# bayespy/bayespy

Hardware: AMD Instinct MI355X
Metric: VB iterations/sec, PCA N=10000000 D=128 K=32 (higher is better)
Workload: dtype f64

## Files before the change

bayespy_amd/csrc/vmp_pca.hip:

```cpp
#include "vmp_common.h"
#include "vmp_stop_rule.h"

namespace {

constexpr int TN = 32;
constexpr int SZ = TN + 2;
constexpr int NT = 256;
constexpr int MAX_KP = 64;
constexpr int MAX_DP = 256;

inline int pow2_blocks(int x, int unit)
{
    int b = (x + unit - 1) / unit;
    int p = 1;
    while (p < b) p <<= 1;
    return p;
}

inline void fill_layout(int D, int K, vmp_pca_layout *L)
{
    const int64_t DP = 32 * pow2_blocks(D, 32);
    const int64_t KP = 16 * pow2_blocks(K, 16);
    int64_t o = 0;
    L->DP = DP;
// ... 1101 lines not shown
        return VMP_PCA_SWEEPS_NOT_BUILT;
    if (vmp_pca_sweep_covered(D, K) != VMP_OK) return VMP_PCA_SWEEPS_NOT_BUILT;
    VMP_REQUIRE(ctx, ring && order, VMP_ERR_INVALID, "null pointer argument");
    VMP_REQUIRE(ctx, n >= 1 && n <= VMP_PCA_MAX_SWEEPS, VMP_ERR_INVALID,
                "between 1 and %d sweeps per call", VMP_PCA_MAX_SWEEPS);
    VMP_REQUIRE(ctx, norder >= 1 && norder <= VMP_BOUND_MAX_ORDER, VMP_ERR_INVALID,
                "between 1 and %d bound terms", VMP_BOUND_MAX_ORDER);
    for (int i = 0; i < norder; ++i)
        VMP_REQUIRE(ctx, order[i] >= -1 && order[i] < VMP_BOUND_TERMS, VMP_ERR_INVALID,
                    "bound term %d out of range", order[i]);
    VMP_REQUIRE(ctx, lay == 0 || lay == 1 || lay == 3, VMP_ERR_INVALID, "unknown layout %d", lay);
    VMP_REQUIRE(ctx, x_prec > 0 && a0_tau > 0 && b0_tau > 0 && a0_alpha > 0 && b0_alpha > 0,
                VMP_ERR_INVALID, "x_prec and the Gamma prior parameters must be positive");
    int32_t rc;
    if (lay == 0) {
        rc = check_pass_args(ctx, Y, X, state, workspace, ldy, ldx, N, D, K);
        if (rc != VMP_OK) return rc;
    } else {
        VMP_REQUIRE(ctx, Y && X && state && workspace && N >= 0, VMP_ERR_INVALID,
                    "null pointer argument");
        VMP_REQUIRE(ctx, ((uintptr_t)Y % 16) == 0 && ((uintptr_t)X % 16) == 0, VMP_ERR_INVALID,
                    "tile-major arrays must be 16-byte aligned");
        if (lay == 1)
            VMP_REQUIRE(ctx, (ldx % 2) == 0 && ldx >= (N + TN - 1) / TN * TN && ldx < (int64_t)170000000,
                        VMP_ERR_INVALID, "row-major X beside a tile-major Y needs KP rows of an even "
                        "leading dimension >= 32 ceil(N/32) (ldx=%lld)", (long long)ldx);
    }
    rc = vmp_pca_ensure_gram(ctx);
    if (rc != VMP_OK) return rc;
    if (!ctx->sweep_ctl) {
        VMP_HIP_CHECK(ctx, hipMalloc(&ctx->sweep_ctl, VMP_SWEEP_CTL_LEN * sizeof(double)));
        VMP_HIP_CHECK(ctx, hipMemsetAsync(ctx->sweep_ctl, 0, VMP_SWEEP_CTL_LEN * sizeof(double),
                                          ctx->stream));
    }
    vmp_pca_layout L;
    fill_layout(D, K, &L);
    double *P = reinterpret_cast<double *>(workspace);
    vmp_sweep_tail t;
    t.P = P;
    t.nb = (int)(L.DP / GR);
    t.ctl = ctx->sweep_ctl;
    t.compare = compare ? 1 : 0;
    t.l0 = l0;
    t.tol = tol;
    t.norder = norder;
    for (int i = 0; i < 8; ++i) t.order[i] = i < norder ? order[i] : -1;
    const bool ticket = n > 1 && ((uintptr_t)state % 16) == 0 &&
                        vmp_tune_get("pca_sweep_ticket", env_int("VMP_PCA_SWEEP_TICKET", 1, 0, 1));
    int wide = vmp_tune_get("pca_sweep_wide", env_int("VMP_PCA_SWEEP_WIDE", 1, 0, 1)) ? 1 : 0;
    if (wide && vmp_tune_get("pca_sweep_local_pxx", env_int("VMP_PCA_SWEEP_LOCAL_PXX", 1, 0, 1)))
        wide = 2;
    if (wide == 2 && vmp_tune_get("pca_sweep_defer", env_int("VMP_PCA_SWEEP_DEFER", 1, 0, 1)))
        wide = 3;
    if (ticket && wide == 3) {
        rc = vmp_pca_sweep_constants(ctx, D, K, n_total, x_prec, a0_tau, b0_tau, a0_alpha, b0_alpha);
        if (rc != VMP_OK) return rc;
    }
    const int stamp_level = ticket ? vmp_tune_get("pca_sweep_stamps", 0) : 0;
    const bool stamps = stamp_level != 0;
    if (stamps) {
        const size_t bytes = (size_t)VMP_PCA_MAX_SWEEPS * VMP_SWEEP_NSTAMP * sizeof(unsigned long long);
        if (!ctx->sweep_stamps) VMP_HIP_CHECK(ctx, hipMalloc(&ctx->sweep_stamps, bytes));
        VMP_HIP_CHECK(ctx, hipMemsetAsync(ctx->sweep_stamps, 0,
                                          (size_t)(n - 1) * VMP_SWEEP_NSTAMP * sizeof(unsigned long long),
                                          ctx->stream));
        ctx->sweep_stamp_rows = n - 1;
    }
    if (ticket) {
        if (!ctx->sweep_tickets) {
            VMP_HIP_CHECK(ctx, hipMalloc(&ctx->sweep_tickets,
                                         VMP_PCA_MAX_SWEEPS * sizeof(unsigned int)));
            VMP_HIP_CHECK(ctx, hipMemsetAsync(ctx->sweep_tickets, 0,
                                              VMP_PCA_MAX_SWEEPS * sizeof(unsigned int), ctx->stream));
        }
    }
    bool head_wide = ticket && wide;
    if (head_wide && ctx->x_pending) {
        head_wide = hipEventQuery(ctx->ev_xdone) == hipSuccess;
        (void)hipGetLastError();
    }
    for (int i = 0; i < n; ++i) {
        const double *stop = i == 0 ? nullptr : ctx->sweep_ctl;
        const bool last = i + 1 == n;
        if (i == 0 && head_wide) {
            rc = vmp_pca_launch_sweep_head_wide(ctx, D, K, n_total, x_prec, a0_tau, b0_tau, a0_alpha,
                                                b0_alpha, state);
            if (rc != VMP_OK) return rc;
        } else if (!ticket || i == 0) {
            rc = vmp_pca_launch_sweep_head(ctx, D, K, n_total, x_prec, a0_tau, b0_tau, a0_alpha,
                                           b0_alpha, state, stop);
            if (rc != VMP_OK) return rc;
        }
        if (last) {
            rc = issue_xpass(ctx, Y, ldy, N, D, K, X, ldx, state, workspace, lay);
            if (rc != VMP_OK) return rc;
        } else {
            ctx->x_superseded += 1;
        }
        t.slot = ring + (int64_t)i * VMP_PCA_SWEEP_SLOT;
        t.first = i == 0;
        if (ticket && !last) {
            rc = vmp_pca_launch_sweep_mid(ctx, D, K, n_total, x_prec, a0_tau, b0_tau, a0_alpha,
                                          b0_alpha, state, P, t, ctx->sweep_tickets + i, wide,
                                          stamps ? ctx->sweep_stamps + (size_t)i * VMP_SWEEP_NSTAMP
                                                 : nullptr, stamp_level);
            if (rc != VMP_OK) return rc;
            ctx->sweep_mid_launches += 1;
        } else {
            rc = run_gram_stats(ctx, L, D, K, state, P, ctx->stream, stop, false);
            if (rc != VMP_OK) return rc;
            rc = vmp_pca_launch_sweep_tail(ctx, D, K, n_total, x_prec, a0_tau, b0_tau, a0_alpha,
                                           b0_alpha, state, t);
            if (rc != VMP_OK) return rc;
        }
        ctx->sweeps_enqueued += 1;
    }
    return VMP_OK;
}

int32_t vmp_pca_sweep_counts(vmp_ctx *ctx, int64_t *enqueued, int64_t *executed, int64_t *skipped)
{
    VMP_REQUIRE(ctx, ctx, VMP_ERR_INVALID, "null argument");
    double c[VMP_SWEEP_CTL_LEN] = {0.0};
    if (ctx->sweep_ctl) {
        VMP_HIP_CHECK(ctx, hipStreamSynchronize(ctx->stream));
        VMP_HIP_CHECK(ctx, hipMemcpy(c, ctx->sweep_ctl, sizeof(c), hipMemcpyDeviceToHost));
    }
    if (enqueued) *enqueued = ctx->sweeps_enqueued;
    if (executed) *executed = (int64_t)c[VMP_SWEEP_EXECUTED];
    if (skipped) *skipped = (int64_t)c[VMP_SWEEP_SKIPPED];
    return VMP_OK;
}

int32_t vmp_pca_sweep_mid_count(vmp_ctx *ctx, int64_t *launches)
{
    VMP_REQUIRE(ctx, ctx && launches, VMP_ERR_INVALID, "null argument");
    *launches = ctx->sweep_mid_launches;
    return VMP_OK;
}

int32_t vmp_pca_sweep_stamps(vmp_ctx *ctx, uint64_t *out, int32_t max_rows, int32_t *rows,
                             int32_t *allocated)
{
    VMP_REQUIRE(ctx, ctx && rows && max_rows >= 0 && (out || max_rows == 0), VMP_ERR_INVALID,
                "null argument");
    if (allocated) *allocated = ctx->sweep_stamps ? 1 : 0;
    *rows = 0;
    if (!ctx->sweep_stamps) return VMP_OK;
    const int n = ctx->sweep_stamp_rows < max_rows ? ctx->sweep_stamp_rows : max_rows;
    if (n > 0) {
        VMP_HIP_CHECK(ctx, hipStreamSynchronize(ctx->stream));
        VMP_HIP_CHECK(ctx, hipMemcpy(out, ctx->sweep_stamps,
                                     (size_t)n * VMP_SWEEP_NSTAMP * sizeof(unsigned long long),
                                     hipMemcpyDeviceToHost));
    }
    *rows = n;
    return VMP_OK;
}

int32_t vmp_pca_gram_stats_form(vmp_ctx *ctx, int32_t D, int32_t K, double *state, void *workspace,
                                int32_t form)
{
    VMP_REQUIRE(ctx, ctx && state && workspace, VMP_ERR_INVALID, "null argument");
    vmp_pca_layout L;
    const int32_t rc = vmp_pca_get_layout(D, K, &L);
    VMP_REQUIRE(ctx, rc == VMP_OK, rc, "unsupported dims D=%d K=%d", D, K);
    double *P = reinterpret_cast<double *>(workspace);
    if (form == 0) return run_gram_stats(ctx, L, D, K, state, P, ctx->stream, nullptr, false);
    VMP_REQUIRE(ctx, form == 1 || form == 2, VMP_ERR_INVALID, "form %d (0, 1 or 2)", form);
    return vmp_pca_launch_gram_fast(ctx, D, K, state, P, form == 2);
}

int32_t vmp_pca_last_pass_ms(vmp_ctx *ctx, double *ms_pass, double *ms_reduce)
{
    VMP_REQUIRE(ctx, ctx != nullptr, VMP_ERR_INVALID, "null argument");
    {
        const int32_t rch = vmp_pca_launch_held(ctx);
        if (rch != VMP_OK) return rch;
    }
    VMP_REQUIRE(ctx, ctx->timing && ctx->ev[0] && ctx->ev_n > 0, VMP_ERR_INVALID,
                "no timed pass (vmp_ctx_set_timing)");
    hipEvent_t *e = ctx->ev + 3 * ((ctx->ev_n - 1) % VMP_EV_RING);
    VMP_HIP_CHECK(ctx, hipEventSynchronize(e[2]));
    float a = 0.f, b = 0.f;
    VMP_HIP_CHECK(ctx, hipEventElapsedTime(&a, e[0], e[1]));
    VMP_HIP_CHECK(ctx, hipEventElapsedTime(&b, e[1], e[2]));
    if (ms_pass) *ms_pass = a;
    if (ms_reduce) *ms_reduce = b;
    return VMP_OK;
}

}
```

bayespy_amd/csrc/vmp_pca_small.hip:

```cpp
#include "vmp_common.h"
#include "vmp_sweep.h"
#include "vmp_stop_rule.h"

#include <stdlib.h>
#include <string.h>
#include <type_traits>

namespace {


struct small_args {
    vmp_pca_layout L;
    int D, K;
    double n_total, x_prec, a0t, b0t, a0a, b0a;
    int has_mean;
};

__device__ inline double ww_centred(const small_args &a, const double *st, int k)
{
    const vmp_pca_layout &L = a.L;
    double v = st[L.off_Sww + k * L.KP + k];
    if (a.has_mean) v += st[L.off_mstat + L.KP + k] - 2.0 * st[L.off_mstat + k];
    return v;
}
// ... 623 lines not shown
#pragma unroll
    for (int b = 0; b < NB; ++b)
#pragma unroll
        for (int m = 0; m < NLB; ++m) {
            const int e = tid + m * NTF;
            const int r = b * RB + e / KP, k = e % KP;
            wv[b][m] = (r < D && k < K) ? st[L.off_W + r * KP + k] : 0.0;
        }
#pragma unroll
    for (int b = 0; b < NB; ++b) {
        if (b < nb) {
#pragma unroll
            for (int m = 0; m < NLB; ++m) {
                const int e = tid + m * NTF;
                SWb[(e / KP) * LDM + (e % KP)] = wv[b][m];
            }
            __syncthreads();
#pragma unroll
            for (int t = 0; t < WT; ++t) {
                const int tile = w + 4 * t;
                if (tile < TPB) {
                    const int tk = tile % KT, td = tile / KT;
                    const v4f64 acc = wave_tile_mma(M + tk * 16 * LDM, LDM, 1, SWb + td * 16 * LDM, 1,
                                                    LDM, KP);
#pragma unroll
                    for (int r = 0; r < 4; ++r) {
                        const int k = tk * 16 + l4 + 4 * r, d = b * RB + td * 16 + l15;
                        if (k < K && d < D) st[L.off_A + k * DP + d] = tau * acc[r];
                    }
                }
            }
            __syncthreads();
        }
    }
    if (tid == 0) {
        st[L.off_scal + 1] = logdet;
        if (bad) st[L.off_scal + 3] = (double)VMP_ERR_NOT_POSDEF;
    }
    stamp.drain();
    stamp(SP_H_A);
}

template <int KP>
__global__ void __launch_bounds__(NTF, 5)
pca_head_fast_kernel(small_args a, double *st, const double *stop)
{
    if (stop && stop[VMP_SWEEP_STOP] != 0.0) return;
    pca_head_body<KP, false>(a, st, nullptr, nullptr, nullptr, 0.0);
}

constexpr int GB = 32;
constexpr int GRA = 8;
constexpr int TAIL_PLAIN = 0, TAIL_GRAM = 1, TAIL_SWEEP = 2;
template <int KP>
struct alignas(16) tail_lds {
    double Sw[KP * (KP + 1)];
    double Cx[KP * (KP + 1)];
    double Sx[KP * (KP + 1)];
    double al[4 * KP];
    double sc[8];
    double red[NTF / 64 + 1];
    double stop;
};
static_assert(sizeof(tail_lds<16>) % 16 == 0 && sizeof(tail_lds<32>) % 16 == 0, "tail_lds size");
template <int KP, int MODE, bool WIDE = false, class STAMP = stamps_off, bool LOCAL = false,
          bool DEFER = false>
__device__ __forceinline__ void pca_tail_body(const small_args &a, double *st, const vmp_sweep_tail *sw,
                                              tail_lds<KP> &s, double *SW = nullptr,
                                              const STAMP &stamp = STAMP(), const double *AL = nullptr)
{
    static_assert(!WIDE || MODE == TAIL_SWEEP, "the wide tail is a sweep tail");
    static_assert(!LOCAL || WIDE, "sum <x><x>^T is formed locally by the wide tail only");
    static_assert(!DEFER || LOCAL, "the bound is deferred behind the local wide tail only");
    constexpr bool GRAM = (MODE == TAIL_GRAM);
    constexpr int LDM = KP + 1, E = KP * KP / NTF;
    extern __shared__ __align__(16) double gl[];
    double *Sw = s.Sw, *Cx = s.Cx, *Sx = s.Sx, *al = s.al, *sc = s.sc, *red = s.red;
    const lay32 L(a.L);
    const int tid = threadIdx.x, D = a.D, K = a.K;
    if constexpr (MODE == TAIL_SWEEP && !LOCAL) {
        if (!sw->first && sw->ctl[VMP_SWEEP_STOP] != 0.0) {
            if (tid == 0) {
                sw->slot[7] = 0.0;
                sw->ctl[VMP_SWEEP_SKIPPED] += 1.0;
            }
            return;
        }
    }
    __builtin_amdgcn_s_setprio(3);
    double t1 = 0.0;
    double sxx[E];
#pragma unroll
    for (int m = 0; m < E; ++m) sxx[m] = 0.0;
    constexpr int NW = WIDE ? FAST_D * KP / NTF : 1;
    double ww[NW], wy[NW], es0[WIDE ? E : 1], es1[WIDE ? E : 1];
    if constexpr (WIDE) {
        const int n = D * KP;
#pragma unroll
        for (int j = 0; j < NW; ++j) {
            const int e = tid + j * NTF;
            ww[j] = e < n ? st[L.off_W + e] : 0.0;
            wy[j] = e < n ? st[L.off_S + e] : 0.0;
        }
#pragma unroll
        for (int m = 0; m < E; ++m) {
            const int e = tid + m * NTF;
            const int i = e / KP, j = e % KP;
            const bool in = (i < K && j < K);
            es0[m] = in ? st[L.off_Sww + i * KP + j] : 0.0;
            es1[m] = in ? st[L.off_CX + i * KP + j] : 0.0;
        }
    }
    if constexpr (LOCAL) {
    } else if constexpr (WIDE) {
        constexpr int NBM = FAST_D / 8;
        const int nb = sw->nb, nb4 = nb & ~3;
        double pv[E][NBM];
#pragma unroll
        for (int m = 0; m < E; ++m)
#pragma unroll
            for (int b = 0; b < NBM; ++b)
                pv[m][b] = b < nb ? sw->P[tid + m * NTF + b * (KP * KP)] : 0.0;
#pragma unroll
        for (int m = 0; m < E; ++m) {
            double s0 = 0.0, s1 = 0.0, s2 = 0.0, s3 = 0.0;
#pragma unroll
// ... 87 lines not shown
            const int i = e / KP, j = e % KP;
            const bool in = (i < K && j < K);
            if constexpr (WIDE) {
                v0[m] = es0[m];
                v1[m] = es1[m];
            } else {
                v0[m] = in ? st[L.off_Sww + i * KP + j] : 0.0;
                v1[m] = in ? st[L.off_CX + i * KP + j] : 0.0;
            }
            if constexpr (MODE != TAIL_PLAIN) v2[m] = in ? sxx[m] : 0.0;
            else v2[m] = in ? st[L.off_S + (L.DP + i) * KP + j] : 0.0;
        }
        if (tid == 0) {
            sc[4] = st[L.off_Syy];
            sc[5] = st[L.off_scal + 0];
            sc[6] = st[L.off_scal + 1];
        }
#pragma unroll
        for (int m = 0; m < E; ++m) {
            const int e = tid + m * NTF;
            const int i = e / KP, j = e % KP;
            Sw[i * LDM + j] = v0[m];
            Cx[i * LDM + j] = v1[m];
            if constexpr (!LOCAL) Sx[i * LDM + j] = v2[m];
        }
    }
    if constexpr (WIDE) {
        const int n = D * KP, jn = (n + 8 * NTF - 1) / (8 * NTF) * 8;
        const int nsw = LOCAL ? L.DP * KP : (D + 31) / 32 * 32 * KP;
#pragma unroll
        for (int j = 0; j < NW; ++j) {
            const int e = tid + j * NTF;
            if (j < jn) t1 += ww[j] * wy[j];
            if (e < nsw) SW[(e / KP) * LDM + (e % KP)] = (e < n && e % KP < K) ? wy[j] : 0.0;
        }
    } else if constexpr (!GRAM) {
        const int n = D * KP;
#pragma unroll 1
        for (int e0 = 0; e0 < n; e0 += 8 * NTF) {
            double w[8], y[8];
#pragma unroll
            for (int m = 0; m < 8; ++m) {
                const int e = e0 + tid + m * NTF;
                w[m] = e < n ? st[L.off_W + e] : 0.0;
                y[m] = e < n ? st[L.off_S + e] : 0.0;
            }
#pragma unroll
            for (int m = 0; m < 8; ++m) t1 += w[m] * y[m];
        }
    }
    (void)ww; (void)wy; (void)es0; (void)es1;
    __syncthreads();
    stamp(SP_T_LOADS);
    if constexpr (LOCAL) {
        constexpr int B = KP / 16;
        const int LA = L.DP + 2;
        const int ki = tid >> 4, ji = tid & 15;
        const int nb = sw->nb, nb4 = nb & ~3;
        const double *ar = AL + ki * LA, *sr = SW + ji;
        double acc[4][B][B];
#pragma unroll
        for (int q = 0; q < 4; ++q)
#pragma unroll
            for (int i = 0; i < B; ++i)
#pragma unroll
                for (int j = 0; j < B; ++j) acc[q][i][j] = 0.0;
        const auto group = [&](int b, double (&p)[B][B]) {
#pragma unroll
            for (int i = 0; i < B; ++i)
#pragma unroll
                for (int j = 0; j < B; ++j) p[i][j] = 0.0;
#pragma unroll
            for (int r = 0; r < GRA; r += 2) {
                v2f64 x[B];
                double y0[B], y1[B];
#pragma unroll
                for (int i = 0; i < B; ++i)
                    x[i] = *reinterpret_cast<const v2f64 *>(ar + 16 * i * LA + b * GRA + r);
#pragma unroll
                for (int j = 0; j < B; ++j) {
                    y0[j] = sr[(b * GRA + r) * LDM + 16 * j];
                    y1[j] = sr[(b * GRA + r + 1) * LDM + 16 * j];
                }
#pragma unroll
                for (int i = 0; i < B; ++i)
#pragma unroll
                    for (int j = 0; j < B; ++j) {
                        p[i][j] = __builtin_fma(x[i][0], y0[j], p[i][j]);
                        p[i][j] = __builtin_fma(x[i][1], y1[j], p[i][j]);
                    }
            }
        };
        double p[B][B];
#pragma unroll 1
        for (int b = 0; b < nb4; b += 4) {
#pragma unroll
            for (int q = 0; q < 4; ++q) {
                group(b + q, p);
#pragma unroll
                for (int i = 0; i < B; ++i)
#pragma unroll
                    for (int j = 0; j < B; ++j) acc[q][i][j] += p[i][j];
            }
        }
#pragma unroll 1
        for (int b = nb4; b < nb; ++b) {
            group(b, p);
// ... 218 lines not shown
        const double *a0 = As + k0 * LA, *a1 = As + (k0 + H) * LA;
        double s00 = 0.0, s01 = 0.0, s10 = 0.0, s11 = 0.0;
#pragma unroll 4
        for (int d = 0; d < D; ++d) {
            const double x0 = g0[d], x1 = g1[d], y0 = a0[d], y1 = a1[d];
            s00 = __builtin_fma(x0, y0, s00);
            s01 = __builtin_fma(x0, y1, s01);
            s10 = __builtin_fma(x1, y0, s10);
            s11 = __builtin_fma(x1, y1, s11);
        }
        Ss[ra * LDS_S + k0] = s00;
        Ss[ra * LDS_S + k0 + H] = s01;
        Ss[(ra + 4) * LDS_S + k0] = s10;
        Ss[(ra + 4) * LDS_S + k0 + H] = s11;
        double *So = st + L.off_S;
        if (r0 + ra < D) {
            if (k0 < K) So[(r0 + ra) * KP + k0] = s00;
            if (k0 + H < K) So[(r0 + ra) * KP + k0 + H] = s01;
        }
        if (r0 + ra + 4 < D) {
            if (k0 < K) So[(r0 + ra + 4) * KP + k0] = s10;
            if (k0 + H < K) So[(r0 + ra + 4) * KP + k0 + H] = s11;
        }
    }
    __syncthreads();
    stamp(SP_SYX);
    double *Pb = P + (int64_t)blk * KP * KP;
#pragma unroll
    for (int m = 0; m < E; ++m) {
        const int e = tid + m * NTF;
        const int k = e / KP, k2 = e % KP;
        double s = 0.0;
        if (k < K && k2 < K) {
#pragma unroll
            for (int r = 0; r < GRA; ++r) s = __builtin_fma(As[k * LA + r0 + r], Ss[r * LDS_S + k2], s);
        }
        Pb[e] = s;
    }
}

template <int KP>
__global__ void __launch_bounds__(NTF)
pca_gram_fast_kernel(vmp_pca_layout L, int D, int K, double *st, double *P)
{
    extern __shared__ __align__(16) double gl[];
    gram_phase_a<KP>(L, D, K, st, P, gl, blockIdx.x);
}

__host__ __device__ inline size_t gram_phase_a_wide_lds(int KP, int DP)
{
    return ((size_t)KP * (DP + 2) + (size_t)GRA * DP + (size_t)GRA * (KP + 1)) * sizeof(double);
}

template <int KP, class STAMP = stamps_off, bool PXX = true>
__device__ __forceinline__ void gram_phase_a_wide(const vmp_pca_layout &L, int D, int K, double *st,
                                                  double *P, double *lds, int blk,
                                                  const STAMP &stamp = STAMP())
{
    constexpr int LDS_S = KP + 1, KT = KP / 16, E = KP * KP / NTF;
    constexpr int NA = KP * (FAST_D / 2) / NTF, NG = GRA * (FAST_D / 2) / NTF;
    const int DP = (int)L.DP, LA = DP + 2;
    const int DP2 = DP >> 1, sh = __builtin_ctz(DP2);
    double *As = lds;
    double *Gs = As + KP * LA;
    double *Ss = Gs + GRA * DP;
    const int tid = threadIdx.x;
    const int r0 = blk * GRA;
    const double *A = st + L.off_A;
    const double *G = st + L.off_G + (int64_t)r0 * DP;
    v2f64 av[NA], gv[NG];
#pragma unroll
    for (int m = 0; m < NA; ++m) {
        const int e = tid + m * NTF;
        const int k = e >> sh, c = (e & (DP2 - 1)) * 2;
        av[m] = *reinterpret_cast<const v2f64 *>(A + (k < K ? k : K - 1) * DP + c);
    }
#pragma unroll
    for (int m = 0; m < NG; ++m) {
        const int e = tid + m * NTF;
        gv[m] = *reinterpret_cast<const v2f64 *>(G + 2 * (e < GRA * DP2 ? e : GRA * DP2 - 1));
    }
#pragma unroll
    for (int m = 0; m < NA; ++m) {
        const int e = tid + m * NTF;
        const int k = e >> sh, c = (e & (DP2 - 1)) * 2;
        if (e < KP * DP2) *reinterpret_cast<v2f64 *>(As + k * LA + c) = k < K ? av[m] : v2f64{0.0, 0.0};
    }
#pragma unroll
    for (int m = 0; m < NG; ++m) {
        const int e = tid + m * NTF;
        if (e < GRA * DP2) *reinterpret_cast<v2f64 *>(Gs + 2 * e) = gv[m];
    }
    __syncthreads();
    stamp(SP_LDS_FILLED);
    {
        const int w = tid >> 6, l = tid & 63;
        if (w < 2 * KT) {
            const int k = (l & 15) + 16 * (w % KT), r = (l >> 4) + 4 * (w / KT);
            const double *g = Gs + r * DP, *ar = As + k * LA;
            double s = 0.0;
#pragma unroll 16
            for (int d = 0; d < D; ++d) s = __builtin_fma(g[d], ar[d], s);
            Ss[r * LDS_S + k] = s;
            if (r0 + r < D && k < K) st[L.off_S + (r0 + r) * KP + k] = s;
        }
    }
    __syncthreads();
    stamp(SP_SYX);
    if constexpr (PXX) {
        double *Pb = P + (int64_t)blk * KP * KP;
#pragma unroll
        for (int m = 0; m < E; ++m) {
            const int e = tid + m * NTF;
            const int k = e / KP, k2 = e % KP;
            double s = 0.0;
            if (k < K && k2 < K) {
#pragma unroll
                for (int r = 0; r < GRA; ++r)
                    s = __builtin_fma(As[k * LA + r0 + r], Ss[r * LDS_S + k2], s);
            }
            Pb[e] = s;
        }
    }
}

template <int KP>
__global__ void __launch_bounds__(NTF)
pca_gram_wide_kernel(vmp_pca_layout L, int D, int K, double *st, double *P)
{
    extern __shared__ __align__(16) double gl[];
    gram_phase_a_wide<KP>(L, D, K, st, P, gl, blockIdx.x);
}

template <int KP, class STAMP>
struct defer_side {
    const small_args &a;
    double *st;
    const vmp_sweep_tail &sw;
    tail_lds<KP> &s;
    const double *sf;
    const STAMP &stamp;
    __device__ __forceinline__ void operator()() const
    {
        constexpr int LDM = KP + 1;
        if (threadIdx.x >= 128) return;
        const lay32 L(a.L);
        const int l = threadIdx.x - 64, D = a.D, K = a.K;
        const bool isa = l < K;
        const int k = isa ? l : 0;
        const double a0 = isa ? a.a0a : a.a0t, b0 = isa ? a.b0a : a.b0t;
        const double av = isa ? s.al[0 * KP + k] : s.sc[0];
        const double bv = isa ? s.al[1 * KP + k] : s.sc[1];
        const double mean = isa ? s.al[2 * KP + k] : s.sc[2];
        const double *c = sf + (isa ? VMP_SWEEP_SF_ALPHA : VMP_SWEEP_SF_TAU);
        const double dg = c[0], lga = c[1], lga0 = c[2], logb0 = c[3];
        const double logb = sf_log(bv);
        const double logx = dg - logb;
        const double g_p = a0 * logb0 - lga0;
        const double g_q = av * logb - lga;
        const double g = g_p - g_q + (bv - b0) * mean + (a0 - av) * logx;
        if (isa) st[L.off_alpha + 3 * KP + k] = logx;
        if (l == 32) st[L.off_tau + 3] = logx;
        stamp.side(SP_S_STATE);
        const double sla = 0.0 + wave_sum(isa ? logx : 0.0);
        const double saw = 0.0 + wave_sum(isa ? mean * s.Sw[k * LDM + k] : 0.0);
        const double lal = 0.0 + wave_sum(isa ? g : 0.0);
        const double logtau = __shfl(logx, 32, 64), Lt = __shfl(g, 32, 64);
        if (l == 0) {
            const double tau = s.sc[2], resid = s.red[0], trx = s.red[1];
            const double Dd = (double)D, Kd = (double)K;
            const double LY = Dd * a.n_total * (-0.5 * sf[VMP_SWEEP_SF_LOG2PI] + 0.5 * logtau)
                              - 0.5 * tau * resid;
            const double LX = -0.5 * a.x_prec * trx
                              + a.n_total * (0.5 * Kd * sf[VMP_SWEEP_SF_LOGXPREC] - 0.5 * s.sc[6] + 0.5 * Kd);
            const double LW = 0.5 * Dd * sla - 0.5 * saw + Dd * (-0.5 * s.sc[5] + 0.5 * Kd);
            st[L.off_L + 0] = LY;
            st[L.off_L + 1] = LX;
            st[L.off_L + 2] = LW;
            st[L.off_L + 3] = Lt;
            st[L.off_L + 4] = lal;
            st[L.off_L + 5] = LY + LX + LW + Lt + lal;
            const double status = !(s.sc[1] > 0.0) ? (double)VMP_ERR_FLOATING : st[L.off_scal + 3];
            double *slot = sw.slot;
            slot[0] = LY;
// ... 116 lines not shown
    }
    __syncthreads();
    stamp(SP_H_SWW);
#pragma unroll
    for (int m = 0; m < E; ++m) {
        const int e = tid + m * NTF;
        const int i = e / KP, j = e % KP;
        double x = (i == j) ? 1.0 : 0.0;
        if (i < K && j < K) {
            x = tau * 0.5 * (T[i * LDM + j] + T[j * LDM + i]);
            if (i == j) x += a.x_prec;
        }
        M[i * LDM + j] = x;
    }
    const auto pad = [&]() {
        if (D == nr && K == KP) return;
        for (int e = tid - 64; e < nr * KP; e += NTF - 64)
            if (e / KP >= D || e % KP >= K) SW[(e / KP) * LDM + (e % KP)] = 0.0;
    };
    sweep_inverse<KP>(M, K, &logdet, &bad, pad);
    stamp(SP_H_INV2);
#pragma unroll
    for (int m = 0; m < E; ++m) {
        const int e = tid + m * NTF;
        const int i = e / KP, j = e % KP;
        if (i < K && j < K) st[L.off_CX + i * KP + j] = M[i * LDM + j];
    }
#pragma unroll
    for (int t = 0; t < WT; ++t) {
        const int tile = w + 4 * t;
        if (tile < nt) {
            const int tk = tile % KT, td = tile / KT;
            const v4f64 acc = wave_tile_mma(M + tk * 16 * LDM, LDM, 1, SW + td * 16 * LDM, 1, LDM, KP);
#pragma unroll
            for (int r = 0; r < 4; ++r) {
                const int k = tk * 16 + l4 + 4 * r, d = td * 16 + l15;
                if (k < K && d < D) st[L.off_A + k * DP + d] = tau * acc[r];
            }
        }
    }
    if (tid == 0) {
        st[L.off_scal + 1] = logdet;
        if (bad) st[L.off_scal + 3] = (double)VMP_ERR_NOT_POSDEF;
    }
    stamp.drain();
    stamp(SP_H_A);
}

__host__ __device__ inline size_t sweep_local_lds(int KP, int DP)
{
    return ((size_t)KP * (DP + 2) + (size_t)DP * (KP + 1) + 2) * sizeof(double);
}

template <int KP, bool WIDE, bool LOCAL, bool DEFER, class STAMP>
__device__ __forceinline__ void pca_sweep_mid_body(const small_args &a, double *st, double *P,
                                                   const vmp_sweep_tail &sw, unsigned int *ticket,
                                                   const double *sf, const STAMP &stamp)
{
    static_assert(!LOCAL || WIDE, "sum <x><x>^T is formed locally beside the wide bodies only");
    static_assert(!DEFER || LOCAL, "the bound is deferred behind the local wide tail only");
    extern __shared__ __align__(16) double gl[];
    __shared__ tail_lds<KP> ts;
    const int tid = threadIdx.x;
    if (!sw.first && sw.ctl[VMP_SWEEP_STOP] != 0.0) {
        if (blockIdx.x == 0 && tid == 0) {
            sw.slot[7] = 0.0;
            sw.ctl[VMP_SWEEP_SKIPPED] += 1.0;
        }
        return;
    }
    stamp(SP_ENTRY);
    if constexpr (WIDE)
        gram_phase_a_wide<KP, STAMP, !LOCAL>(a.L, a.D, a.K, st, P, gl, blockIdx.x, stamp);
    else
        gram_phase_a<KP>(a.L, a.D, a.K, st, P, gl, blockIdx.x, stamp);
    asm volatile("s_waitcnt vmcnt(0)" ::: "memory");
    __syncthreads();
    stamp(SP_PXX);
    const int na = LOCAL ? KP * ((int)a.L.DP + 2) : 0;
    double *SW = gl + na;
    unsigned int *word = reinterpret_cast<unsigned int *>(LOCAL ? SW + (int)a.L.DP * (KP + 1) : gl);
    if (tid == 0) {
        __builtin_amdgcn_fence(__ATOMIC_RELEASE, "agent");
        asm volatile("s_waitcnt vmcnt(0)" ::: "memory");
        *word = __hip_atomic_fetch_add(ticket, 1u, __ATOMIC_RELAXED, __HIP_MEMORY_SCOPE_AGENT);
    }
    __syncthreads();
    if (*word != gridDim.x - 1) return;
    stamp(SP_TICKET);
    if (tid == 0) {
        __builtin_amdgcn_fence(__ATOMIC_ACQUIRE, "agent");
        asm volatile("s_waitcnt vmcnt(0)" ::: "memory");
        *ticket = 0u;
    }
    __syncthreads();
    stamp(SP_ACQUIRE);
    pca_tail_body<KP, TAIL_SWEEP, WIDE, STAMP, LOCAL, DEFER>(a, st, &sw, ts, SW, stamp, gl);
    __syncthreads();
    if constexpr (DEFER) {
        const defer_side<KP, STAMP> side{a, st, sw, ts, sf, stamp};
        pca_head_wide<KP>(a, st, ts.Cx, ts.Sx, ts.al + 2 * KP, ts.sc[2], SW, stamp, side, &ts.stop);
        return;
    }
    if (ts.stop != 0.0) return;
    if constexpr (WIDE)
        pca_head_wide<KP>(a, st, ts.Cx, ts.Sx, ts.al + 2 * KP, ts.sc[2], SW, stamp);
    else
        pca_head_body<KP, true>(a, st, ts.Cx, ts.Sx, ts.al + 2 * KP, ts.sc[2], stamp);
}

template <int KP, bool WIDE, bool LOCAL, bool DEFER = false>
__global__ void __launch_bounds__(NTF)
pca_sweep_mid_kernel(small_args a, double *st, double *P, vmp_sweep_tail sw, unsigned int *ticket,
                     const double *sf)
{
    pca_sweep_mid_body<KP, WIDE, LOCAL, DEFER>(a, st, P, sw, ticket, sf, stamps_off());
}

template <int KP, bool WIDE, bool LOCAL, bool DEFER = false>
__global__ void __launch_bounds__(NTF)
pca_sweep_mid_stamped_kernel(small_args a, double *st, double *P, vmp_sweep_tail sw,
                             unsigned int *ticket, const double *sf, unsigned long long *out, int level)
{
    __shared__ unsigned long long stl[VMP_SWEEP_NSTAMP];
    if (threadIdx.x < VMP_SWEEP_NSTAMP) stl[threadIdx.x] = 0;
    __syncthreads();
    const stamps_on stamp{stl, level};
    pca_sweep_mid_body<KP, WIDE, LOCAL, DEFER>(a, st, P, sw, ticket, sf, stamp);
    if (threadIdx.x == 0 && stl[SP_T_LOADS] != 0)
        for (int i = 0; i < VMP_SWEEP_NSTAMP; ++i) out[i] = stl[i];
}

template <int KP>
__global__ void __launch_bounds__(NTF)
pca_head_wide_kernel(small_args a, double *st)
{
    constexpr int LDM = KP + 1, E = KP * KP / NTF, NW = FAST_D * KP / NTF;
    __shared__ __align__(16) double M[KP * LDM], T[KP * LDM], SW[FAST_D * LDM], alm[KP];
    const lay32 L(a.L);
    const int tid = threadIdx.x, D = a.D, K = a.K;
    const int n = D * KP, nsw = (D + 31) / 32 * 32 * KP;
    double cx[E], sx[E], wy[NW];
#pragma unroll
    for (int m = 0; m < E; ++m) {
        const int e = tid + m * NTF;
        const int i = e / KP, j = e % KP;
        const bool in = (i < K && j < K);
        cx[m] = in ? st[L.off_CX + i * KP + j] : 0.0;
        sx[m] = in ? st[L.off_S + (L.DP + i) * KP + j] : 0.0;
    }
#pragma unroll
    for (int j = 0; j < NW; ++j) {
        const int e = tid + j * NTF;
        wy[j] = (e < n && e % KP < K) ? st[L.off_S + e] : 0.0;
    }
    const double tau = st[L.off_tau + 2];
    if (tid < KP) alm[tid] = tid < K ? st[L.off_alpha + 2 * KP + tid] : 0.0;
#pragma unroll
    for (int m = 0; m < E; ++m) {
        const int e = tid + m * NTF;
        M[(e / KP) * LDM + (e % KP)] = cx[m];
        T[(e / KP) * LDM + (e % KP)] = sx[m];
    }
#pragma unroll
    for (int j = 0; j < NW; ++j) {
        const int e = tid + j * NTF;
        if (e < nsw) SW[(e / KP) * LDM + (e % KP)] = wy[j];
    }
    __syncthreads();
    pca_head_wide<KP>(a, st, M, T, alm, tau, SW, stamps_off());
}

__global__ void __launch_bounds__(64)
pca_sweep_sf_kernel(small_args a, double *sf)
{
    const int l = threadIdx.x;
    if (l >= VMP_SWEEP_SF_LEN) return;
    const double ta = a.a0t + 0.5 * (double)a.D * a.n_total;
    const double aa = a.a0a + 0.5 * (double)a.D;
    double v;
    switch (l) {
// ... 161 lines not shown

int32_t vmp_pca_launch_sweep_head(vmp_ctx *ctx, int32_t D, int32_t K, int64_t n_total, double x_prec,
                                  double a0t, double b0t, double a0a, double b0a, double *state,
                                  const double *stop)
{
    small_args a;
    const int32_t rc = fill_small_args(ctx, a, D, K, n_total, x_prec, a0t, b0t, a0a, b0a);
    if (rc != VMP_OK) return rc;
    if (a.L.KP == 16)
        hipLaunchKernelGGL(pca_head_fast_kernel<16>, dim3(1), dim3(NTF), 0, ctx->stream, a, state, stop);
    else
        hipLaunchKernelGGL(pca_head_fast_kernel<32>, dim3(1), dim3(NTF), 0, ctx->stream, a, state, stop);
    VMP_HIP_CHECK(ctx, hipGetLastError());
    return VMP_OK;
}

int32_t vmp_pca_launch_sweep_tail(vmp_ctx *ctx, int32_t D, int32_t K, int64_t n_total, double x_prec,
                                  double a0t, double b0t, double a0a, double b0a, double *state,
                                  const vmp_sweep_tail &t)
{
    small_args a;
    const int32_t rc = fill_small_args(ctx, a, D, K, n_total, x_prec, a0t, b0t, a0a, b0a);
    if (rc != VMP_OK) return rc;
    if (a.L.KP == 16)
        hipLaunchKernelGGL(pca_tail_sweep_kernel<16>, dim3(1), dim3(NTF), 0, ctx->stream, a, state, t);
    else
        hipLaunchKernelGGL(pca_tail_sweep_kernel<32>, dim3(1), dim3(NTF), 0, ctx->stream, a, state, t);
    VMP_HIP_CHECK(ctx, hipGetLastError());
    return VMP_OK;
}

template <typename F>
static int32_t raise_lds_once(vmp_ctx *ctx, F *k16, F *k32, bool *raised)
{
    const int dev = ctx->device & 63;
    if (raised[dev]) return VMP_OK;
    VMP_HIP_CHECK(ctx, hipFuncSetAttribute((const void *)k16,
                                           hipFuncAttributeMaxDynamicSharedMemorySize, 96 * 1024));
    VMP_HIP_CHECK(ctx, hipFuncSetAttribute((const void *)k32,
                                           hipFuncAttributeMaxDynamicSharedMemorySize, 96 * 1024));
    raised[dev] = true;
    return VMP_OK;
}

int32_t vmp_pca_launch_gram_fast(vmp_ctx *ctx, int32_t D, int32_t K, double *state, double *P,
                                 int32_t wide)
{
    vmp_pca_layout L;
    const int32_t rc = vmp_pca_get_layout(D, K, &L);
    VMP_REQUIRE(ctx, rc == VMP_OK, rc, "unsupported dims D=%d K=%d", D, K);
    VMP_REQUIRE(ctx, L.KP <= 32 && D <= FAST_D, VMP_ERR_UNSUPPORTED,
                "the fast Gram statistics cover K <= 32, D <= %d", FAST_D);
    VMP_REQUIRE(ctx, ((uintptr_t)state % 16) == 0, VMP_ERR_INVALID, "state must be 16-byte aligned");
    static bool raised[2][64] = {{false}};
    const int32_t rr = wide ? raise_lds_once(ctx, pca_gram_wide_kernel<16>, pca_gram_wide_kernel<32>,
                                             raised[1])
                            : raise_lds_once(ctx, pca_gram_fast_kernel<16>, pca_gram_fast_kernel<32>,
                                             raised[0]);
    if (rr != VMP_OK) return rr;
    const int nb = (int)(L.DP / GRA);
    if (wide) {
        const size_t ldw = gram_phase_a_wide_lds((int)L.KP, (int)L.DP);
        if (L.KP == 16)
            hipLaunchKernelGGL(pca_gram_wide_kernel<16>, dim3(nb), dim3(NTF), ldw, ctx->stream, L, D, K,
                               state, P);
        else
            hipLaunchKernelGGL(pca_gram_wide_kernel<32>, dim3(nb), dim3(NTF), ldw, ctx->stream, L, D, K,
                               state, P);
        VMP_HIP_CHECK(ctx, hipGetLastError());
        return VMP_OK;
    }
    const size_t lds = gram_phase_a_lds((int)L.KP, (int)L.DP);
    if (L.KP == 16)
        hipLaunchKernelGGL(pca_gram_fast_kernel<16>, dim3(nb), dim3(NTF), lds, ctx->stream, L, D, K,
                           state, P);
    else
        hipLaunchKernelGGL(pca_gram_fast_kernel<32>, dim3(nb), dim3(NTF), lds, ctx->stream, L, D, K,
                           state, P);
    VMP_HIP_CHECK(ctx, hipGetLastError());
    return VMP_OK;
}

template <int KP, bool WIDE, bool LOCAL, bool DEFER = false>
static int32_t launch_mid(vmp_ctx *ctx, const small_args &a, double *state, double *P,
                          const vmp_sweep_tail &t, unsigned int *ticket, unsigned long long *stamps,
                          int stamp_level)
{
    VMP_REQUIRE(ctx, !DEFER || ctx->sweep_sf, VMP_ERR_INVALID,
                "the deferred sweep needs vmp_pca_sweep_constants first");
    static bool raised[2][64] = {{false}};
    const int dev = ctx->device & 63, s = stamps ? 1 : 0;
    if (!raised[s][dev]) {
        const void *f = stamps ? (const void *)pca_sweep_mid_stamped_kernel<KP, WIDE, LOCAL, DEFER>
                               : (const void *)pca_sweep_mid_kernel<KP, WIDE, LOCAL, DEFER>;
        VMP_HIP_CHECK(ctx, hipFuncSetAttribute(f, hipFuncAttributeMaxDynamicSharedMemorySize,
                                               96 * 1024));
        raised[s][dev] = true;
    }
    const size_t lds = LOCAL ? sweep_local_lds((int)a.L.KP, (int)a.L.DP)
                       : WIDE ? gram_phase_a_wide_lds((int)a.L.KP, (int)a.L.DP)
                              : gram_phase_a_lds((int)a.L.KP, (int)a.L.DP);
    const dim3 nb((unsigned)(a.L.DP / GRA));
    if (stamps)
        hipLaunchKernelGGL((pca_sweep_mid_stamped_kernel<KP, WIDE, LOCAL, DEFER>), nb, dim3(NTF), lds,
                           ctx->stream, a, state, P, t, ticket, (const double *)ctx->sweep_sf, stamps,
                           stamp_level);
    else
        hipLaunchKernelGGL((pca_sweep_mid_kernel<KP, WIDE, LOCAL, DEFER>), nb, dim3(NTF), lds, ctx->stream, a,
                           state, P, t, ticket, (const double *)ctx->sweep_sf);
    VMP_HIP_CHECK(ctx, hipGetLastError());
    return VMP_OK;
}

int32_t vmp_pca_launch_sweep_mid(vmp_ctx *ctx, int32_t D, int32_t K, int64_t n_total, double x_prec,
                                 double a0t, double b0t, double a0a, double b0a, double *state,
                                 double *P, const vmp_sweep_tail &t, unsigned int *ticket, int32_t wide,
                                 unsigned long long *stamps, int32_t stamp_level)
{
    small_args a;
    const int32_t rc = fill_small_args(ctx, a, D, K, n_total, x_prec, a0t, b0t, a0a, b0a);
    if (rc != VMP_OK) return rc;
    const int sl = stamp_level;
    if (a.L.KP == 16)
        return wide == 3 ? launch_mid<16, true, true, true>(ctx, a, state, P, t, ticket, stamps, sl)
               : wide == 2 ? launch_mid<16, true, true>(ctx, a, state, P, t, ticket, stamps, sl)
               : wide      ? launch_mid<16, true, false>(ctx, a, state, P, t, ticket, stamps, sl)
                           : launch_mid<16, false, false>(ctx, a, state, P, t, ticket, stamps, sl);
    return wide == 3 ? launch_mid<32, true, true, true>(ctx, a, state, P, t, ticket, stamps, sl)
           : wide == 2 ? launch_mid<32, true, true>(ctx, a, state, P, t, ticket, stamps, sl)
           : wide      ? launch_mid<32, true, false>(ctx, a, state, P, t, ticket, stamps, sl)
                       : launch_mid<32, false, false>(ctx, a, state, P, t, ticket, stamps, sl);
}

int32_t vmp_pca_sweep_constants(vmp_ctx *ctx, int32_t D, int32_t K, int64_t n_total, double x_prec,
                                double a0t, double b0t, double a0a, double b0a)
{
    small_args a;
    const int32_t rc = fill_small_args(ctx, a, D, K, n_total, x_prec, a0t, b0t, a0a, b0a);
    if (rc != VMP_OK) return rc;
    const double key[7] = {a0t, b0t, a0a, b0a, (double)D, (double)n_total, x_prec};
    if (ctx->sweep_sf && ctx->sweep_sf_valid && memcmp(key, ctx->sweep_sf_key, sizeof(key)) == 0)
        return VMP_OK;
    if (!ctx->sweep_sf) VMP_HIP_CHECK(ctx, hipMalloc(&ctx->sweep_sf, VMP_SWEEP_SF_LEN * sizeof(double)));
    ctx->sweep_sf_valid = 0;
    hipLaunchKernelGGL(pca_sweep_sf_kernel, dim3(1), dim3(64), 0, ctx->stream, a, ctx->sweep_sf);
    VMP_HIP_CHECK(ctx, hipGetLastError());
    memcpy(ctx->sweep_sf_key, key, sizeof(key));
    ctx->sweep_sf_valid = 1;
    return VMP_OK;
}

int32_t vmp_pca_launch_sweep_head_wide(vmp_ctx *ctx, int32_t D, int32_t K, int64_t n_total,
                                       double x_prec, double a0t, double b0t, double a0a, double b0a,
                                       double *state)
{
    small_args a;
    const int32_t rc = fill_small_args(ctx, a, D, K, n_total, x_prec, a0t, b0t, a0a, b0a);
    if (rc != VMP_OK) return rc;
    if (a.L.KP == 16)
        hipLaunchKernelGGL(pca_head_wide_kernel<16>, dim3(1), dim3(NTF), 0, ctx->stream, a, state);
    else
        hipLaunchKernelGGL(pca_head_wide_kernel<32>, dim3(1), dim3(NTF), 0, ctx->stream, a, state);
    VMP_HIP_CHECK(ctx, hipGetLastError());
    return VMP_OK;
}

extern "C" {

int32_t vmp_pca_small_ops(vmp_ctx *ctx, int32_t D, int32_t K, int64_t n_total, double x_prec,
                          double a0_tau, double b0_tau, double a0_alpha, double b0_alpha,
                          int32_t nops, const int32_t *ops, double *state)
{
    return launch_small(ctx, D, K, n_total, x_prec, a0_tau, b0_tau, a0_alpha, b0_alpha, nops, ops,
                        state);
}

int32_t vmp_pca_small_ops_mean(vmp_ctx *ctx, int32_t D, int32_t K, int64_t n_total, double x_prec,
                               double a0_tau, double b0_tau, double a0_alpha, double b0_alpha,
                               int32_t nops, const int32_t *ops, int32_t has_mean, double *state)
{
    return launch_small(ctx, D, K, n_total, x_prec, a0_tau, b0_tau, a0_alpha, b0_alpha, nops, ops,
// ... 40 lines not shown
```

Measured before the change: 26070.

## Add lean sweep path with padded Gram staging and register-tiled local Pxx

Adds a LEAN variant of the deferred wide sweep-mid kernel, on by default. It pads the staged Gram rows in LDS to stride DP+2 and reads them as v2f64 pairs in the A·G dot products, to cut LDS bank conflicts and load count. For KP=32 it also replaces the local sum <x><x>^T loop with a 4x4 register-tiled accumulation, reduced across lanes with DPP row swaps and shuffles. It exposes a standalone lean Gram kernel as form 3. The cost is a slightly larger LDS footprint, more register pressure and more template variants.

Result: no change. 26040 (median of 2 runs) (-0.1%).

```diff
diff --git a/bayespy_amd/csrc/vmp_pca.hip b/bayespy_amd/csrc/vmp_pca.hip
--- a/bayespy_amd/csrc/vmp_pca.hip
+++ b/bayespy_amd/csrc/vmp_pca.hip
@@ -1177,6 +1177,7 @@
         wide = 2;
     if (wide == 2 && vmp_tune_get("pca_sweep_defer", env_int("VMP_PCA_SWEEP_DEFER", 1, 0, 1)))
         wide = 3;
+    const bool lean = wide == 3 && vmp_tune_get("pca_sweep_lean", env_int("VMP_PCA_SWEEP_LEAN", 1, 0, 1));
     if (ticket && wide == 3) {
         rc = vmp_pca_sweep_constants(ctx, D, K, n_total, x_prec, a0_tau, b0_tau, a0_alpha, b0_alpha);
         if (rc != VMP_OK) return rc;
@@ -1226,7 +1227,8 @@
         t.first = i == 0;
         if (ticket && !last) {
             rc = vmp_pca_launch_sweep_mid(ctx, D, K, n_total, x_prec, a0_tau, b0_tau, a0_alpha,
-                                          b0_alpha, state, P, t, ctx->sweep_tickets + i, wide,
+                                          b0_alpha, state, P, t, ctx->sweep_tickets + i,
+                                          lean ? 4 : wide,
                                           stamps ? ctx->sweep_stamps + (size_t)i * VMP_SWEEP_NSTAMP
                                                  : nullptr, stamp_level);
             if (rc != VMP_OK) return rc;
@@ -1292,8 +1294,8 @@
     VMP_REQUIRE(ctx, rc == VMP_OK, rc, "unsupported dims D=%d K=%d", D, K);
     double *P = reinterpret_cast<double *>(workspace);
     if (form == 0) return run_gram_stats(ctx, L, D, K, state, P, ctx->stream, nullptr, false);
-    VMP_REQUIRE(ctx, form == 1 || form == 2, VMP_ERR_INVALID, "form %d (0, 1 or 2)", form);
-    return vmp_pca_launch_gram_fast(ctx, D, K, state, P, form == 2);
+    VMP_REQUIRE(ctx, form >= 1 && form <= 3, VMP_ERR_INVALID, "form %d (0, 1, 2 or 3)", form);
+    return vmp_pca_launch_gram_fast(ctx, D, K, state, P, form - 1);
 }
 
 int32_t vmp_pca_last_pass_ms(vmp_ctx *ctx, double *ms_pass, double *ms_reduce)
diff --git a/bayespy_amd/csrc/vmp_pca_small.hip b/bayespy_amd/csrc/vmp_pca_small.hip
--- a/bayespy_amd/csrc/vmp_pca_small.hip
+++ b/bayespy_amd/csrc/vmp_pca_small.hip
@@ -699,6 +699,13 @@
 constexpr int GB = 32;
 constexpr int GRA = 8;
 constexpr int TAIL_PLAIN = 0, TAIL_GRAM = 1, TAIL_SWEEP = 2;
+__device__ __forceinline__ double row_swap8(double v)
+{
+    const int lo = __builtin_amdgcn_mov_dpp(__double2loint(v), 0x128, 0xf, 0xf, true);
+    const int hi = __builtin_amdgcn_mov_dpp(__double2hiint(v), 0x128, 0xf, 0xf, true);
+    return __hiloint2double(hi, lo);
+}
+
 template <int KP>
 struct alignas(16) tail_lds {
     double Sw[KP * (KP + 1)];
@@ -711,7 +718,7 @@
 };
 static_assert(sizeof(tail_lds<16>) % 16 == 0 && sizeof(tail_lds<32>) % 16 == 0, "tail_lds size");
 template <int KP, int MODE, bool WIDE = false, class STAMP = stamps_off, bool LOCAL = false,
-          bool DEFER = false>
+          bool DEFER = false, bool LEAN = false>
 __device__ __forceinline__ void pca_tail_body(const small_args &a, double *st, const vmp_sweep_tail *sw,
                                               tail_lds<KP> &s, double *SW = nullptr,
                                               const STAMP &stamp = STAMP(), const double *AL = nullptr)
@@ -719,6 +726,7 @@
     static_assert(!WIDE || MODE == TAIL_SWEEP, "the wide tail is a sweep tail");
     static_assert(!LOCAL || WIDE, "sum <x><x>^T is formed locally by the wide tail only");
     static_assert(!DEFER || LOCAL, "the bound is deferred behind the local wide tail only");
+    static_assert(!LEAN || DEFER, "the lean loops belong to the deferred form");
     constexpr bool GRAM = (MODE == TAIL_GRAM);
     constexpr int LDM = KP + 1, E = KP * KP / NTF;
     extern __shared__ __align__(16) double gl[];
@@ -912,7 +920,71 @@
     (void)ww; (void)wy; (void)es0; (void)es1;
     __syncthreads();
     stamp(SP_T_LOADS);
-    if constexpr (LOCAL) {
+    if constexpr (LOCAL && LEAN && KP == 32) {
+        const int LA = L.DP + 2;
+        const int bj = tid & 7, q = (tid >> 3) & 3, bi = tid >> 5;
+        const int nb = sw->nb;
+        double acc[4][4], p[4][4];
+#pragma unroll
+        for (int i = 0; i < 4; ++i)
+#pragma unroll
+            for (int j = 0; j < 4; ++j) acc[i][j] = 0.0;
+#pragma unroll 1
+        for (int b = q; b < nb; b += 4) {
+            const double *ar = AL + bi * LA + b * GRA, *sr = SW + b * GRA * LDM + bj;
+#pragma unroll
+            for (int i = 0; i < 4; ++i)
+#pragma unroll
+                for (int j = 0; j < 4; ++j) p[i][j] = 0.0;
+#pragma unroll
+            for (int r = 0; r < GRA; r += 2) {
+                v2f64 x[4];
+                double y0[4], y1[4];
+#pragma unroll
+                for (int i = 0; i < 4; ++i)
+                    x[i] = *reinterpret_cast<const v2f64 *>(ar + 8 * i * LA + r);
+#pragma unroll
+                for (int j = 0; j < 4; ++j) {
+                    y0[j] = sr[r * LDM + 8 * j];
+                    y1[j] = sr[(r + 1) * LDM + 8 * j];
+                }
+#pragma unroll
+                for (int i = 0; i < 4; ++i)
+#pragma unroll
+                    for (int j = 0; j < 4; ++j) {
+                        p[i][j] = __builtin_fma(x[i][0], y0[j], p[i][j]);
+                        p[i][j] = __builtin_fma(x[i][1], y1[j], p[i][j]);
+                    }
+            }
+#pragma unroll
+            for (int i = 0; i < 4; ++i)
+#pragma unroll
+                for (int j = 0; j < 4; ++j) acc[i][j] += p[i][j];
+        }
+        const bool up = (q & 2) != 0;
+        double fin[2][4];
+#pragma unroll
+        for (int i = 0; i < 4; ++i)
+#pragma unroll
+            for (int j = 0; j < 4; ++j) acc[i][j] += row_swap8(acc[i][j]);
+#pragma unroll
+        for (int i = 0; i < 2; ++i)
+#pragma unroll
+            for (int j = 0; j < 4; ++j) {
+                const double give = up ? acc[i][j] : acc[i + 2][j], keep = up ? acc[i + 2][j] : acc[i][j];
+                fin[i][j] = keep + __shfl_xor(give, 16, 64);
+            }
+#pragma unroll
+        for (int j = 0; j < 4; ++j) {
+            const int k = bi + 8 * q, k2 = bj + 8 * j;
+            const double v = (q & 1) ? fin[1][j] : fin[0][j];
+            const double x = (k < K && k2 < K) ? v : 0.0;
+            st[L.off_S + (L.DP + k) * KP + k2] = x;
+            Sx[k * LDM + k2] = x;
+        }
+        __syncthreads();
+        stamp(SP_T_PXX);
+    } else if constexpr (LOCAL) {
         constexpr int B = KP / 16;
         const int LA = L.DP + 2;
         const int ki = tid >> 4, ji = tid & 15;
@@ -1237,18 +1309,23 @@
     return ((size_t)KP * (DP + 2) + (size_t)GRA * DP + (size_t)GRA * (KP + 1)) * sizeof(double);
 }
 
-template <int KP, class STAMP = stamps_off, bool PXX = true>
+__host__ __device__ inline size_t gram_phase_a_lean_lds(int KP, int DP)
+{
+    return gram_phase_a_wide_lds(KP, DP) + (size_t)GRA * 2 * sizeof(double);
+}
+
+template <int KP, class STAMP = stamps_off, bool PXX = true, bool LEAN = false>
 __device__ __forceinline__ void gram_phase_a_wide(const vmp_pca_layout &L, int D, int K, double *st,
                                                   double *P, double *lds, int blk,
                                                   const STAMP &stamp = STAMP())
 {
     constexpr int LDS_S = KP + 1, KT = KP / 16, E = KP * KP / NTF;
     constexpr int NA = KP * (FAST_D / 2) / NTF, NG = GRA * (FAST_D / 2) / NTF;
-    const int DP = (int)L.DP, LA = DP + 2;
+    const int DP = (int)L.DP, LA = DP + 2, LG = LEAN ? DP + 2 : DP;
     const int DP2 = DP >> 1, sh = __builtin_ctz(DP2);
     double *As = lds;
     double *Gs = As + KP * LA;
-    double *Ss = Gs + GRA * DP;
+    double *Ss = Gs + GRA * LG;
     const int tid = threadIdx.x;
     const int r0 = blk * GRA;
     const double *A = st + L.off_A;
@@ -1274,7 +1351,11 @@
 #pragma unroll
     for (int m = 0; m < NG; ++m) {
         const int e = tid + m * NTF;
-        if (e < GRA * DP2) *reinterpret_cast<v2f64 *>(Gs + 2 * e) = gv[m];
+        if constexpr (LEAN) {
+            if (e < GRA * DP2) *reinterpret_cast<v2f64 *>(Gs + (e >> sh) * LG + (e & (DP2 - 1)) * 2) = gv[m];
+        } else {
+            if (e < GRA * DP2) *reinterpret_cast<v2f64 *>(Gs + 2 * e) = gv[m];
+        }
     }
     __syncthreads();
     stamp(SP_LDS_FILLED);
@@ -1282,10 +1363,23 @@
         const int w = tid >> 6, l = tid & 63;
         if (w < 2 * KT) {
             const int k = (l & 15) + 16 * (w % KT), r = (l >> 4) + 4 * (w / KT);
-            const double *g = Gs + r * DP, *ar = As + k * LA;
+            const double *g = Gs + r * LG, *ar = As + k * LA;
             double s = 0.0;
+            if constexpr (LEAN) {
+                const v2f64 *g2 = reinterpret_cast<const v2f64 *>(g);
+                const v2f64 *a2 = reinterpret_cast<const v2f64 *>(ar);
+                const int D2 = D >> 1;
+#pragma unroll 8
+                for (int j = 0; j < D2; ++j) {
+                    const v2f64 x = g2[j], y = a2[j];
+                    s = __builtin_fma(x[0], y[0], s);
+                    s = __builtin_fma(x[1], y[1], s);
+                }
+                if (D & 1) s = __builtin_fma(g[D - 1], ar[D - 1], s);
+            } else {
 #pragma unroll 16
-            for (int d = 0; d < D; ++d) s = __builtin_fma(g[d], ar[d], s);
+                for (int d = 0; d < D; ++d) s = __builtin_fma(g[d], ar[d], s);
+            }
             Ss[r * LDS_S + k] = s;
             if (r0 + r < D && k < K) st[L.off_S + (r0 + r) * KP + k] = s;
         }
@@ -1315,6 +1409,14 @@
 {
     extern __shared__ __align__(16) double gl[];
     gram_phase_a_wide<KP>(L, D, K, st, P, gl, blockIdx.x);
+}
+
+template <int KP>
+__global__ void __launch_bounds__(NTF)
+pca_gram_lean_kernel(vmp_pca_layout L, int D, int K, double *st, double *P)
+{
+    extern __shared__ __align__(16) double gl[];
+    gram_phase_a_wide<KP, stamps_off, true, true>(L, D, K, st, P, gl, blockIdx.x);
 }
 
 template <int KP, class STAMP>
@@ -1537,7 +1639,7 @@
     return ((size_t)KP * (DP + 2) + (size_t)DP * (KP + 1) + 2) * sizeof(double);
 }
 
-template <int KP, bool WIDE, bool LOCAL, bool DEFER, class STAMP>
+template <int KP, bool WIDE, bool LOCAL, bool DEFER, bool LEAN, class STAMP>
 __device__ __forceinline__ void pca_sweep_mid_body(const small_args &a, double *st, double *P,
                                                    const vmp_sweep_tail &sw, unsigned int *ticket,
                                                    const double *sf, const STAMP &stamp)
@@ -1556,7 +1658,7 @@
     }
     stamp(SP_ENTRY);
     if constexpr (WIDE)
-        gram_phase_a_wide<KP, STAMP, !LOCAL>(a.L, a.D, a.K, st, P, gl, blockIdx.x, stamp);
+        gram_phase_a_wide<KP, STAMP, !LOCAL, LEAN>(a.L, a.D, a.K, st, P, gl, blockIdx.x, stamp);
     else
         gram_phase_a<KP>(a.L, a.D, a.K, st, P, gl, blockIdx.x, stamp);
     asm volatile("s_waitcnt vmcnt(0)" ::: "memory");
@@ -1580,7 +1682,7 @@
     }
     __syncthreads();
     stamp(SP_ACQUIRE);
-    pca_tail_body<KP, TAIL_SWEEP, WIDE, STAMP, LOCAL, DEFER>(a, st, &sw, ts, SW, stamp, gl);
+    pca_tail_body<KP, TAIL_SWEEP, WIDE, STAMP, LOCAL, DEFER, LEAN>(a, st, &sw, ts, SW, stamp, gl);
     __syncthreads();
     if constexpr (DEFER) {
         const defer_side<KP, STAMP> side{a, st, sw, ts, sf, stamp};
@@ -1594,15 +1696,15 @@
         pca_head_body<KP, true>(a, st, ts.Cx, ts.Sx, ts.al + 2 * KP, ts.sc[2], stamp);
 }
 
-template <int KP, bool WIDE, bool LOCAL, bool DEFER = false>
+template <int KP, bool WIDE, bool LOCAL, bool DEFER = false, bool LEAN = false>
 __global__ void __launch_bounds__(NTF)
 pca_sweep_mid_kernel(small_args a, double *st, double *P, vmp_sweep_tail sw, unsigned int *ticket,
                      const double *sf)
 {
-    pca_sweep_mid_body<KP, WIDE, LOCAL, DEFER>(a, st, P, sw, ticket, sf, stamps_off());
-}
-
-template <int KP, bool WIDE, bool LOCAL, bool DEFER = false>
+    pca_sweep_mid_body<KP, WIDE, LOCAL, DEFER, LEAN>(a, st, P, sw, ticket, sf, stamps_off());
+}
+
+template <int KP, bool WIDE, bool LOCAL, bool DEFER = false, bool LEAN = false>
 __global__ void __launch_bounds__(NTF)
 pca_sweep_mid_stamped_kernel(small_args a, double *st, double *P, vmp_sweep_tail sw,
                              unsigned int *ticket, const double *sf, unsigned long long *out, int level)
@@ -1611,7 +1713,7 @@
     if (threadIdx.x < VMP_SWEEP_NSTAMP) stl[threadIdx.x] = 0;
     __syncthreads();
     const stamps_on stamp{stl, level};
-    pca_sweep_mid_body<KP, WIDE, LOCAL, DEFER>(a, st, P, sw, ticket, sf, stamp);
+    pca_sweep_mid_body<KP, WIDE, LOCAL, DEFER, LEAN>(a, st, P, sw, ticket, sf, stamp);
     if (threadIdx.x == 0 && stl[SP_T_LOADS] != 0)
         for (int i = 0; i < VMP_SWEEP_NSTAMP; ++i) out[i] = stl[i];
 }
@@ -1879,16 +1981,25 @@
     VMP_REQUIRE(ctx, L.KP <= 32 && D <= FAST_D, VMP_ERR_UNSUPPORTED,
                 "the fast Gram statistics cover K <= 32, D <= %d", FAST_D);
     VMP_REQUIRE(ctx, ((uintptr_t)state % 16) == 0, VMP_ERR_INVALID, "state must be 16-byte aligned");
-    static bool raised[2][64] = {{false}};
-    const int32_t rr = wide ? raise_lds_once(ctx, pca_gram_wide_kernel<16>, pca_gram_wide_kernel<32>,
-                                             raised[1])
-                            : raise_lds_once(ctx, pca_gram_fast_kernel<16>, pca_gram_fast_kernel<32>,
-                                             raised[0]);
+    static bool raised[3][64] = {{false}};
+    const int32_t rr = wide == 2 ? raise_lds_once(ctx, pca_gram_lean_kernel<16>, pca_gram_lean_kernel<32>,
+                                                  raised[2])
+                       : wide    ? raise_lds_once(ctx, pca_gram_wide_kernel<16>, pca_gram_wide_kernel<32>,
+                                                  raised[1])
+                                 : raise_lds_once(ctx, pca_gram_fast_kernel<16>, pca_gram_fast_kernel<32>,
+                                                  raised[0]);
     if (rr != VMP_OK) return rr;
     const int nb = (int)(L.DP / GRA);
     if (wide) {
-        const size_t ldw = gram_phase_a_wide_lds((int)L.KP, (int)L.DP);
-        if (L.KP == 16)
+        const size_t ldw = wide == 2 ? gram_phase_a_lean_lds((int)L.KP, (int)L.DP)
+                                     : gram_phase_a_wide_lds((int)L.KP, (int)L.DP);
+        if (wide == 2 && L.KP == 16)
+            hipLaunchKernelGGL(pca_gram_lean_kernel<16>, dim3(nb), dim3(NTF), ldw, ctx->stream, L, D, K,
+                               state, P);
+        else if (wide == 2)
+            hipLaunchKernelGGL(pca_gram_lean_kernel<32>, dim3(nb), dim3(NTF), ldw, ctx->stream, L, D, K,
+                               state, P);
+        else if (L.KP == 16)
             hipLaunchKernelGGL(pca_gram_wide_kernel<16>, dim3(nb), dim3(NTF), ldw, ctx->stream, L, D, K,
                                state, P);
         else
@@ -1908,7 +2019,7 @@
     return VMP_OK;
 }
 
-template <int KP, bool WIDE, bool LOCAL, bool DEFER = false>
+template <int KP, bool WIDE, bool LOCAL, bool DEFER = false, bool LEAN = false>
 static int32_t launch_mid(vmp_ctx *ctx, const small_args &a, double *state, double *P,
                           const vmp_sweep_tail &t, unsigned int *ticket, unsigned long long *stamps,
                           int stamp_level)
@@ -1918,8 +2029,8 @@
     static bool raised[2][64] = {{false}};
     const int dev = ctx->device & 63, s = stamps ? 1 : 0;
     if (!raised[s][dev]) {
-        const void *f = stamps ? (const void *)pca_sweep_mid_stamped_kernel<KP, WIDE, LOCAL, DEFER>
-                               : (const void *)pca_sweep_mid_kernel<KP, WIDE, LOCAL, DEFER>;
+        const void *f = stamps ? (const void *)pca_sweep_mid_stamped_kernel<KP, WIDE, LOCAL, DEFER, LEAN>
+                               : (const void *)pca_sweep_mid_kernel<KP, WIDE, LOCAL, DEFER, LEAN>;
         VMP_HIP_CHECK(ctx, hipFuncSetAttribute(f, hipFuncAttributeMaxDynamicSharedMemorySize,
                                                96 * 1024));
         raised[s][dev] = true;
@@ -1929,11 +2040,11 @@
                               : gram_phase_a_lds((int)a.L.KP, (int)a.L.DP);
     const dim3 nb((unsigned)(a.L.DP / GRA));
     if (stamps)
-        hipLaunchKernelGGL((pca_sweep_mid_stamped_kernel<KP, WIDE, LOCAL, DEFER>), nb, dim3(NTF), lds,
+        hipLaunchKernelGGL((pca_sweep_mid_stamped_kernel<KP, WIDE, LOCAL, DEFER, LEAN>), nb, dim3(NTF), lds,
                            ctx->stream, a, state, P, t, ticket, (const double *)ctx->sweep_sf, stamps,
                            stamp_level);
     else
-        hipLaunchKernelGGL((pca_sweep_mid_kernel<KP, WIDE, LOCAL, DEFER>), nb, dim3(NTF), lds, ctx->stream, a,
+        hipLaunchKernelGGL((pca_sweep_mid_kernel<KP, WIDE, LOCAL, DEFER, LEAN>), nb, dim3(NTF), lds, ctx->stream, a,
                            state, P, t, ticket, (const double *)ctx->sweep_sf);
     VMP_HIP_CHECK(ctx, hipGetLastError());
     return VMP_OK;
@@ -1949,11 +2060,13 @@
     if (rc != VMP_OK) return rc;
     const int sl = stamp_level;
     if (a.L.KP == 16)
-        return wide == 3 ? launch_mid<16, true, true, true>(ctx, a, state, P, t, ticket, stamps, sl)
+        return wide == 4 ? launch_mid<16, true, true, true, true>(ctx, a, state, P, t, ticket, stamps, sl)
+               : wide == 3 ? launch_mid<16, true, true, true>(ctx, a, state, P, t, ticket, stamps, sl)
                : wide == 2 ? launch_mid<16, true, true>(ctx, a, state, P, t, ticket, stamps, sl)
                : wide      ? launch_mid<16, true, false>(ctx, a, state, P, t, ticket, stamps, sl)
                            : launch_mid<16, false, false>(ctx, a, state, P, t, ticket, stamps, sl);
-    return wide == 3 ? launch_mid<32, true, true, true>(ctx, a, state, P, t, ticket, stamps, sl)
+    return wide == 4 ? launch_mid<32, true, true, true, true>(ctx, a, state, P, t, ticket, stamps, sl)
+           : wide == 3 ? launch_mid<32, true, true, true>(ctx, a, state, P, t, ticket, stamps, sl)
            : wide == 2 ? launch_mid<32, true, true>(ctx, a, state, P, t, ticket, stamps, sl)
            : wide      ? launch_mid<32, true, false>(ctx, a, state, P, t, ticket, stamps, sl)
                        : launch_mid<32, false, false>(ctx, a, state, P, t, ticket, stamps, sl);
```
